# radiocosmology/cora

Hardware: AMD Instinct MI355X
Metric: sky-maps/sec (nside=1024, lmax=2048, 256 freq) (higher is better)
Workload: dtype f64

## Files before the change

### cora_amd/_lib.py

```python
import ctypes
import os
import weakref

import numpy as np

_HERE = os.path.dirname(os.path.abspath(__file__))
LIB_PATH = os.environ.get("CORAHIP_LIB", os.path.join(_HERE, "libcorahip.so"))

c_int, c_double, c_void_p, c_size_t = ctypes.c_int, ctypes.c_double, ctypes.c_void_p, ctypes.c_size_t
c_u64, c_char_p = ctypes.c_uint64, ctypes.c_char_p
PTR = c_void_p

SIGNATURES = {
    "corahip_abi_version": (c_int, []),
    "corahip_abi_minor": (c_int, []),
    "corahip_last_error": (c_char_p, []),
    "corahip_device_count": (c_int, [ctypes.POINTER(c_int)]),
    "corahip_ctx_create": (c_int, [c_int, ctypes.POINTER(c_void_p)]),
    "corahip_ctx_destroy": (c_int, [c_void_p]),
    "corahip_ctx_set_stream": (c_int, [c_void_p, c_void_p]),
    "corahip_ctx_sync": (c_int, [c_void_p]),
    "corahip_timer_begin": (c_int, [c_void_p]),
    "corahip_timer_end": (c_int, [c_void_p, ctypes.POINTER(ctypes.c_float)]),
    "corahip_profile_enable": (c_int, [c_void_p, c_int]),
    "corahip_profile_get": (c_int, [c_void_p, c_char_p, ctypes.POINTER(c_double), ctypes.POINTER(c_int)]),
    "corahip_profile_reset": (c_int, [c_void_p]),
    "corahip_malloc": (c_int, [c_void_p, c_size_t, ctypes.POINTER(c_void_p)]),
    "corahip_free": (c_int, [c_void_p, c_void_p]),
    "corahip_memcpy_h2d": (c_int, [c_void_p, c_void_p, c_void_p, c_size_t]),
    "corahip_memcpy_d2h": (c_int, [c_void_p, c_void_p, c_void_p, c_size_t]),
    "corahip_clarray_table21cm": (c_int, [c_void_p, PTR, PTR, PTR, c_int, c_int, c_double, c_double, c_double,
                                          PTR, PTR, PTR, PTR, c_int, c_int, PTR, PTR, c_int, PTR]),
    "corahip_clarray_table21cm_pairs": (c_int, [c_void_p, PTR, PTR, PTR, c_int, c_int, c_double, c_double, c_double,
                                                PTR, PTR, PTR, PTR, c_int, c_int, PTR, PTR, c_int, c_int, c_int, c_int,
                                                PTR]),
    "corahip_clarray_pairs_finish": (c_int, [c_void_p, PTR, c_int, c_int, c_int, c_int, PTR]),
    "corahip_clarray_tables_pin": (c_int, [c_void_p, PTR, PTR, PTR, c_u64]),
    "corahip_aps_table21cm_points": (c_int, [c_void_p, PTR, PTR, PTR, c_int, c_int, c_double, c_double, c_double,
                                             ctypes.c_long, PTR, PTR, PTR, PTR, PTR, PTR, PTR]),
    "corahip_clarray_separable": (c_int, [c_void_p, PTR, c_int, PTR, c_int, c_int, PTR, PTR]),
    "corahip_romb_reduce": (c_int, [c_void_p, PTR, c_int, c_int, c_int, PTR, PTR]),
    "corahip_factor_batched": (c_int, [c_void_p, PTR, c_int, c_int, c_double, c_double, PTR, PTR]),
    "corahip_normals_philox": (c_int, [c_void_p, c_u64, c_int, c_int, PTR]),
    "corahip_normals_pcg64": (c_int, [c_void_p, ctypes.POINTER(c_u64), ctypes.POINTER(c_u64), ctypes.c_int64, PTR,
                                      ctypes.POINTER(c_u64)]),
    "corahip_normals_mt19937_legacy": (c_int, [c_void_p, c_void_p, ctypes.c_int64, PTR]),
    "corahip_glibc_exp": (c_int, [c_void_p, PTR, ctypes.c_int64, PTR]),
    "corahip_pcg64_advance": (c_int, [ctypes.POINTER(c_u64), ctypes.POINTER(c_u64), c_u64, ctypes.POINTER(c_u64)]),
    "corahip_draw_alm_philox": (c_int, [c_void_p, PTR, PTR, c_u64, c_int, c_int, c_int, c_int, PTR]),
    "corahip_draw_alm_philox_rows": (c_int, [c_void_p, PTR, PTR, c_u64, c_int, c_int, c_int, c_int, PTR]),
    "corahip_draw_alm": (c_int, [c_void_p, PTR, PTR, PTR, c_int, c_int, c_int, c_int, PTR]),
# ... 345 lines not shown

    def to_host(self, t):
        if t.numel() * t.element_size() < self._PINNED_MIN_BYTES:
            return t.cpu().numpy()
        host, done = self.to_host_async(t)
        done.synchronize()
        return host.numpy()

    def pin_tables(self, dd, dv, vv, generation):
        _check(self.lib.corahip_clarray_tables_pin(self.h, self._f64(dd), self._f64(dv), self._f64(vv), c_u64(int(generation))))

    def unpin_tables(self, generation=0):
        if self.h:
            _check(self.lib.corahip_clarray_tables_pin(self.h, None, None, None, c_u64(int(generation))))

    def clarray_table21cm(self, dd, dv, vv, kperpmin, kperpmax, kparmax, chi, pfd, f, b, F, zint, w, log10l):
        nl = log10l.numel()
        out = self.empty((nl, F, F))
        nkperp, nkpar = dd.shape
        _check(self.lib.corahip_clarray_table21cm(
            self.h, self._f64(dd), self._f64(dv), self._f64(vv), nkperp, nkpar, kperpmin, kperpmax, kparmax,
            self._f64(chi), self._f64(pfd), self._f64(f), self._f64(b), F, zint, self._f64(w), self._f64(log10l),
            nl, self._f64(out)))
        return out

    def clarray_table21cm_pairs(self, dd, dv, vv, kperpmin, kperpmax, kparmax, chi, pfd, f, b, F, zint, w, log10l,
                                pair_first, pair_step, l_block, nblocks=None):
        torch = _torch()
        nl = log10l.numel()
        npl = (F * (F + 1) // 2 + pair_step - 1) // pair_step
        nblk = (nl + l_block - 1) // l_block
        if nblocks is not None:
            assert nblocks >= nblk
            nblk = nblocks
        out = torch.zeros((nblk, npl, l_block), dtype=torch.float64, device=self.device)
        nkperp, nkpar = dd.shape
        _check(self.lib.corahip_clarray_table21cm_pairs(
            self.h, self._f64(dd), self._f64(dv), self._f64(vv), nkperp, nkpar, kperpmin, kperpmax, kparmax,
            self._f64(chi), self._f64(pfd), self._f64(f), self._f64(b), F, zint, self._f64(w), self._f64(log10l),
            nl, pair_first, pair_step, l_block, self._f64(out)))
        return out

    def clarray_pairs_finish(self, slabs, F, nl):
        nranks, npl, l_stride = slabs.shape
        assert npl == (F * (F + 1) // 2 + nranks - 1) // nranks and nl <= l_stride
        out = self.empty((nl, F, F))
        _check(self.lib.corahip_clarray_pairs_finish(self.h, self._f64(slabs), F, nranks, l_stride, nl, self._f64(out)))
        return out

    def aps_table21cm_points(self, dd, dv, vv, kperpmin, kperpmax, kparmax, lx, chi1, chi2, cdd, cdv, cvv):
        n = lx.numel()
        out = self.empty((n,))
        nkperp, nkpar = dd.shape
        _check(self.lib.corahip_aps_table21cm_points(
            self.h, self._f64(dd), self._f64(dv), self._f64(vv), nkperp, nkpar, kperpmin, kperpmax, kparmax, n,
            self._f64(lx), self._f64(chi1), self._f64(chi2), self._f64(cdd), self._f64(cdv), self._f64(cvv),
            self._f64(out)))
        return out

    def clarray_separable(self, al, bcov, F, zint, w):
        nl = al.numel()
        out = self.empty((nl, F, F))
# ... 1284 lines not shown
```

### cora_amd/core/maps.py

```python
import numpy as np

from .. import _lib
from ..util import constants
from . import skysim


def _cell_centres(extent, count):
    return (0.5 + np.arange(count)) * (extent / count)


class Map2d(object):

    _geometry_fields = ("x_width", "y_width", "x_num", "y_num", "_nside")

    x_width = y_width = 5.0
    x_num = y_num = 128
    _nside = 128

    @classmethod
    def like_map(cls, mapobj, *args, **kwargs):
        new = cls(*args, **kwargs)
        new._adopt_geometry(mapobj)
        return new

# ... 101 lines not shown
        if self.lmax is None:
            return 3 * self.nside - 1
        return int(self.lmax)

    def _channels(self):
        return np.asarray(self.nu_pixels, dtype=np.float64)

    def getsky(self, rng=None):
        nu = self._channels()
        ctx = _lib.get_context()
        prep = None
        if not isinstance(rng, skysim.DeviceRNG):
            prep = skysim.prepare_numpy_stream(ctx, rng, self._lmax(), len(nu))
        try:
            cl = skysim.clarray_device(self.angular_powerspectrum, self._lmax(), nu,
                                       zromb=self.oversample)
        except BaseException:
            if prep is not None:
                prep.abort()
            raise
        fluct = skysim.mkfullsky_device(cl, self.nside, rng=rng, prepared=prep)
        mean = np.asarray(self.mean_nu(nu), dtype=np.float64) * np.ones(nu.shape)
        if np.any(mean != 0.0):
            fluct += ctx.to_device(mean)[:, None]
        return ctx.to_host(fluct)

    def getpolsky(self, rng=None):
        stokes_i = self.getsky(rng=rng)
        nfreq, npix = stokes_i.shape
        cube = np.zeros((nfreq, 4, npix), dtype=stokes_i.dtype)
        cube[:, 0, :] = stokes_i
        return cube

    def getalms(self, lmax, rng=None):
        cl = skysim.clarray_device(self.angular_powerspectrum, lmax, self._channels())
        return _lib.get_context().to_host(skysim.mkfullsky_device(cl, self.nside, alms=True, rng=rng))
```

### cora_amd/core/skysim.py

```python
import weakref

import numpy as np
import scipy.integrate as si

from .. import _lib
from ..util import nputil
from ..util.nputil import DeviceRNG

_GENERIC_LCHUNK = 8


def romberg_weights(zromb):
    if zromb == 0:
        return np.ones(1)
    zint = 2**zromb + 1
    return si.romb(np.eye(zint), dx=1.0, axis=0) / 2**zromb


def _plan_of(aps):
    obj = getattr(aps, "__self__", None)
    fn = getattr(obj, "_clarray_plan", None)
    return fn(aps) if fn is not None else None


def clarray_device(aps, lmax, zarray, zromb=3, zwidth=None):
    zarray = np.asarray(zarray, dtype=np.float64)
    ctx = _lib.get_context()
    zlen = zarray.size
    if zromb == 0:
        zint = 1
        za = zarray.copy()
    else:
        zsort = np.sort(zarray)
        zhalf = np.abs(zsort[1] - zsort[0]) / 2.0 if zwidth is None else zwidth / 2.0
        zint = 2**zromb + 1
        za = (zarray[:, np.newaxis] + np.linspace(-zhalf, zhalf, zint)[np.newaxis, :]).flatten()
        np.array_split(np.arange(lmax + 1), lmax // 5)
    w = ctx.to_device(romberg_weights(zromb))
    larr = np.arange(lmax + 1, dtype=np.float64)

    plan = _plan_of(aps)
    if plan is not None and plan["kind"] == "table21cm":
        p = plan["prepare"](ctx, za)
        lx = np.log10(np.where(larr == 0.0, 1e-10, larr))
        return ctx.clarray_table21cm(p["dd"], p["dv"], p["vv"], p["kperpmin"], p["kperpmax"], p["kparmax"],
                                     ctx.to_device(p["chi"]), ctx.to_device(p["pfd"]), ctx.to_device(p["f"]),
                                     ctx.to_device(p["b"]), zlen, zint, w, ctx.to_device(lx))
    if plan is not None and plan["kind"] == "separable":
        al, bcov = plan["prepare"](larr.copy(), za)
        return ctx.clarray_separable(ctx.to_device(al), ctx.to_device(bcov), zlen, zint, w)

    import torch

    out = ctx.empty((lmax + 1, zlen, zlen))
    for l0 in range(0, lmax + 1, _GENERIC_LCHUNK):
        lsec = np.arange(l0, min(l0 + _GENERIC_LCHUNK, lmax + 1))
        clt = aps(lsec[:, np.newaxis, np.newaxis].astype(np.float64), za[np.newaxis, :, np.newaxis],
                  za[np.newaxis, np.newaxis, :])
        clt = np.array(np.broadcast_to(clt, (len(lsec), za.size, za.size)), dtype=np.float64, order="C", copy=True)
        out[l0 : l0 + len(lsec)] = ctx.romb_reduce(torch.from_numpy(clt).to(ctx.device), len(lsec), zlen, zint, w)
    return out

# ... 402 lines not shown
```

### cora_amd/csrc/clarray.hip

```cpp
#include "common.h"

#include <cstring>
#include <type_traits>

#define CL_MAXZ 17

#define CL_XS 512
#define CL_LPT 9

__global__ void cl_transpose_kernel(const double *__restrict__ dd, const double *__restrict__ dv,
                                    const double *__restrict__ vv, int nkperp, int nkpar, double *__restrict__ tt) {
    __shared__ double tile[32][33];
    const double *src = blockIdx.z == 0 ? dd : (blockIdx.z == 1 ? dv : vv);
    double *dst = tt + (size_t)blockIdx.z * nkpar * CL_XS;
    const int x0 = blockIdx.y * 32, y0 = blockIdx.x * 32;
    const int tx = threadIdx.x & 31, ty = threadIdx.x >> 5;
    for (int r = ty; r < 32; r += 8) {
        const int x = x0 + r, y = y0 + tx;
        tile[r][tx] = (x < nkperp && y < nkpar) ? src[(size_t)x * nkpar + y] : 0.0;
    }
    __syncthreads();
    for (int r = ty; r < 32; r += 8) {
        const int y = y0 + r, x = x0 + tx;
        if (y < nkpar && x < CL_XS) dst[(size_t)y * CL_XS + x] = (x < nkperp) ? tile[tx][r] : 0.0;
// ... 226 lines not shown
        dd = 4 * xq + (sq & 3);
    } else {
        p -= (long)nfull * CL_BAND;
        int e = n >= CL_BAND ? CL_BAND - 1 : n;
        i = nfull;
        while (p >= e) {
            p -= e;
            e--;
            i++;
        }
        dd = (int)p;
    }
    return make_int2(i, i + CL_BAND * B + dd);
}

__global__ void cl_finish_kernel(const double *__restrict__ scratch, long npairs, int W, long npl, int lstride, int nl,
                                 int F, double *__restrict__ out) {
    __shared__ double tile[32][33];
    const long s0 = (long)blockIdx.x * 32;
    const int l0 = blockIdx.y * 32;
    const int tx = threadIdx.x & 31, ty = threadIdx.x >> 5;
    const long nslot = npl * W;
    for (int r = ty; r < 32; r += 8) {
        const long sl = s0 + r;
        const int l = l0 + tx;
        tile[r][tx] = (sl < nslot && l < nl) ? scratch[(size_t)sl * lstride + l] : 0.0;
    }
    __syncthreads();
    const long sl = s0 + tx;
    const long p = sl < nslot ? (sl % npl) * W + sl / npl : npairs;
    if (p >= npairs) return;
    const int2 ij = pair_of_index(p, F);
    for (int r = ty; r < 32; r += 8) {
        const int l = l0 + r;
        if (l < nl) {
            out[((size_t)l * F + ij.x) * F + ij.y] = tile[tx][r];
        }
    }
}

__global__ void cl_mirror_kernel(double *__restrict__ out, int F) {
    __shared__ double tile[32][33];
    const int nt = (F + 31) / 32;
    int ti = 0, rem = blockIdx.x;
    while (rem >= nt - ti) {
        rem -= nt - ti;
        ti++;
    }
    const int tj = ti + rem;
    double *o = out + (size_t)blockIdx.y * F * F;
    const int tx = threadIdx.x & 31, ty = threadIdx.x >> 5;
    for (int r = ty; r < 32; r += 8) {
        const int i = ti * 32 + r, j = tj * 32 + tx;
        tile[r][tx] = (i < F && j < F) ? o[(size_t)i * F + j] : 0.0;
    }
    __syncthreads();
    for (int r = ty; r < 32; r += 8) {
        const int j = tj * 32 + r, i = ti * 32 + tx;
        if (j < F && i < F && j > i) o[(size_t)j * F + i] = tile[tx][r];
    }
}
static int launch_mirror(corahip_ctx *ctx, double *out, int nl, int F) {
    const int nt = (F + 31) / 32;
    dim3 grid((unsigned)(nt * (nt + 1) / 2), (unsigned)nl);
    cl_mirror_kernel<<<grid, 256, 0, ctx->stream>>>(out, F);
    LAUNCH_CHECK();
    return 0;
}

__global__ void separable_kernel(const double *__restrict__ al, int nl, const double *__restrict__ bcov, int F, int zint,
                                 const double *__restrict__ w, double *__restrict__ out) {
    const long n = (long)nl * F * F;
    const int nz = F * zint;
    for (long q = (long)blockIdx.x * blockDim.x + threadIdx.x; q < n; q += (long)gridDim.x * blockDim.x) {
        const int j = (int)(q % F), i = (int)((q / F) % F);
        const long l = q / ((long)F * F);
        double s = 0.0;
        for (int a = 0; a < zint; a++) {
            double t = 0.0;
            for (int b = 0; b < zint; b++) t += w[b] * bcov[(size_t)(i * zint + a) * nz + j * zint + b];
// ... 97 lines not shown
    ARG_CHECK(ctx != nullptr);
    if (dd == nullptr && generation != 0 && !(ctx->tt_pinned && ctx->tt_pin_gen == generation))
        return 0;
    const bool same = ctx->tt_pinned && dd && ctx->tt_pin[0] == dd && ctx->tt_pin[1] == dv && ctx->tt_pin[2] == vv &&
                      ctx->tt_pin_gen == generation;
    if (same) return 0;
    ctx->tt_pin[0] = dd;
    ctx->tt_pin[1] = dv;
    ctx->tt_pin[2] = vv;
    ctx->tt_pin_gen = generation;
    ctx->tt_pinned = dd != nullptr;
    ctx->tt_valid = false;
    return 0;
}

int corahip_clarray_table21cm(corahip_ctx *ctx, const double *dd, const double *dv, const double *vv, int nkperp,
                              int nkpar, double kperpmin, double kperpmax, double kparmax, const double *chi,
                              const double *pfd, const double *f, const double *b, int F, int zint, const double *w,
                              const double *log10l, int nl, double *out) {
    ARG_CHECK(ctx != nullptr && dd && dv && vv && chi && pfd && f && b && w && log10l && out);
    ARG_CHECK(nkperp >= 2 && nkperp < CL_XS && nkpar >= 2 && F >= 1 && zint >= 1 && zint <= CL_MAXZ && nl >= 1);
    ARG_CHECK(kperpmin > 0 && kperpmax > kperpmin && kparmax > 0);
    StageTimer t(ctx, "clarray");
    const long npairs = (long)F * (F + 1) / 2;
    double *scratch = nullptr;
    int rc;
    if ((rc = corahip_ctx_scratch(ctx, 1, sizeof(double) * (size_t)npairs * nl, (void **)&scratch))) return rc;
    if ((rc = clarray21_pairs(ctx, dd, dv, vv, nkperp, nkpar, kperpmin, kperpmax, kparmax, chi, pfd, f, b, F, zint, w,
                              log10l, nl, 0, 1, npairs, nl, scratch)))
        return rc;
    dim3 grid((unsigned)((npairs + 31) / 32), (nl + 31) / 32);
    cl_finish_kernel<<<grid, 256, 0, ctx->stream>>>(scratch, npairs, 1, npairs, nl, nl, F, out);
    LAUNCH_CHECK();
    return launch_mirror(ctx, out, nl, F);
}

int corahip_clarray_table21cm_pairs(corahip_ctx *ctx, const double *dd, const double *dv, const double *vv, int nkperp,
                                    int nkpar, double kperpmin, double kperpmax, double kparmax, const double *chi,
                                    const double *pfd, const double *f, const double *b, int F, int zint,
                                    const double *w, const double *log10l, int nl, int pair_first, int pair_step,
                                    int l_block, double *out_pairs) {
    ARG_CHECK(ctx != nullptr && dd && dv && vv && chi && pfd && f && b && w && log10l && out_pairs);
    ARG_CHECK(nkperp >= 2 && nkperp < CL_XS && nkpar >= 2 && F >= 1 && zint >= 1 && zint <= CL_MAXZ && nl >= 1);
    ARG_CHECK(kperpmin > 0 && kperpmax > kperpmin && kparmax > 0);
    ARG_CHECK(pair_step >= 1 && pair_first >= 0 && pair_first < pair_step && l_block >= 1);
    StageTimer t(ctx, "clarray");
    const long npairs = (long)F * (F + 1) / 2;
    const long npl = (npairs + pair_step - 1) / pair_step;
    return clarray21_pairs(ctx, dd, dv, vv, nkperp, nkpar, kperpmin, kperpmax, kparmax, chi, pfd, f, b, F, zint, w,
                           log10l, nl, pair_first, pair_step, npl, l_block, out_pairs);
}

int corahip_clarray_pairs_finish(corahip_ctx *ctx, const double *pairs_in, int F, int nranks, int l_stride, int nl,
                                 double *out) {
    ARG_CHECK(ctx != nullptr && pairs_in && out && F >= 1 && nranks >= 1 && nl >= 1 && l_stride >= nl);
    StageTimer t(ctx, "clarray");
    const long npairs = (long)F * (F + 1) / 2;
    const long npl = (npairs + nranks - 1) / nranks;
    dim3 grid((unsigned)((npl * nranks + 31) / 32), (nl + 31) / 32);
    cl_finish_kernel<<<grid, 256, 0, ctx->stream>>>(pairs_in, npairs, nranks, npl, l_stride, nl, F, out);
    LAUNCH_CHECK();
    return launch_mirror(ctx, out, nl, F);
}

int corahip_clarray_separable(corahip_ctx *ctx, const double *al, int nl, const double *bcov, int F, int zint,
                              const double *w, double *out) {
    ARG_CHECK(ctx != nullptr && al && bcov && w && out && nl >= 1 && F >= 1 && zint >= 1);
    StageTimer t(ctx, "clarray");
    const long n = (long)nl * F * F;
    separable_kernel<<<(int)std::min<long>((n + 255) / 256, 4096), 256, 0, ctx->stream>>>(al, nl, bcov, F, zint, w, out);
    LAUNCH_CHECK();
    return 0;
}

int corahip_romb_reduce(corahip_ctx *ctx, const double *clt, int nl, int F, int zint, const double *w, double *out) {
    ARG_CHECK(ctx != nullptr && clt && w && out && nl >= 1 && F >= 1 && zint >= 1);
    StageTimer t(ctx, "clarray");
// ... 23 lines not shown
```

### cora_amd/csrc/common.h

```cpp
#pragma once
#include <hip/hip_runtime.h>

#include <cstdarg>
#include <cstdint>
#include <cstdio>
#include <map>
#include <string>
#include <type_traits>
#include <vector>

#include "../../include/corahip.h"

void corahip_set_error(const char *fmt, ...);

struct corahip_prof_entry {
    double total_ms = 0.0;
    int launches = 0;
};

struct corahip_pending_event {
    std::string name;
    hipEvent_t e0, e1;
};

struct corahip_linefft_plan {
    int n = 0, P = 0, logP = 0, blu = 0;
    int Pct = 0;
    double2 *filt_ct = nullptr;
    double2 *tw = nullptr;
    double2 *chirp = nullptr;
    double2 *filt = nullptr;
    double2 *rtw = nullptr;
};

#define CORAHIP_NSCRATCH 12
struct corahip_ctx {
    int device = 0;
    hipStream_t stream = nullptr;
    hipStream_t stream2 = nullptr;
    hipEvent_t ev_fork = nullptr, ev_join = nullptr;
    int *k5_tickets = nullptr;
    unsigned *draw_slot_tab = nullptr;
    int draw_slot_lmax = -1;
    bool mt_plist_ready = false;
    hipStream_t gen_stream = nullptr;
    hipEvent_t ev_ring[8] = {};
    const void *draw_pending = nullptr;
    hipEvent_t t0 = nullptr, t1 = nullptr;
    bool profile = false;
    std::map<std::string, corahip_prof_entry> prof;
// ... 123 lines not shown
```

### cora_amd/csrc/factor.hip

```cpp
#include "common.h"
#include "jacobi_sweep.h"

#include <algorithm>
#include <vector>

#define CH_NB 32

__global__ void __launch_bounds__(256)
chol_kernel(const double *__restrict__ C, int F, double jitter_rel, double *__restrict__ T,
            int32_t *__restrict__ info) {
    extern __shared__ __attribute__((aligned(16))) double lds[];
    double *D = lds;
    double *PA = lds + CH_NB * (CH_NB + 1);
    double *PB = PA + 64 * (CH_NB + 1);
    double *red = PB + 64 * (CH_NB + 1);
    int *flag = reinterpret_cast<int *>(red + 256);

    const int tid = threadIdx.x;
    const size_t off = (size_t)blockIdx.x * F * F;
    const double *A = C + off;
    double *Tl = T + off;

    double dmax = -INFINITY;
    for (int i = tid; i < F; i += 256) dmax = fmax(dmax, A[(size_t)i * F + i]);
// ... 123 lines not shown
    }
    if (tid == 0) info[blockIdx.x] = *flag;
}

#define CHM_S 34
#ifndef CHM_STAMPS
#define CHM_STAMPS 0
#endif
#if CHM_STAMPS
__device__ unsigned long long g_chm_stamps[8];
#define CSTAMP(k) { unsigned long long _t; asm volatile("s_memtime %0\n\ts_waitcnt lgkmcnt(0)" : "=s"(_t)::"memory"); c_acc[k] += _t - c_last; c_last = _t; }
#else
#define CSTAMP(k)
#endif

template <bool TALL>
__global__ void __launch_bounds__(256)
chol_ll_kernel(const double *__restrict__ C, int F, double jitter_rel, double *__restrict__ T,
               int32_t *__restrict__ info) {
    extern __shared__ __attribute__((aligned(16))) double lds[];
    double *D = lds;
    double *red = lds + CH_NB * (CH_NB + 1);
    int *flag = reinterpret_cast<int *>(red + 256);
    double *rdiag = red + 256 + 2;
    double *stage = rdiag + CH_NB;

    const int tid = threadIdx.x, lane = tid & 63, wave = tid >> 6;
    const int ri = lane & 15, kq = lane >> 4;
    const size_t off = (size_t)blockIdx.x * F * F;
    const double *A = C + off;
    double *Tl = T + off;
    double *PA = stage + (size_t)wave * (TALL ? 1 : 2) * 32 * CHM_S, *PB = PA + 32 * CHM_S;
    double *PBS = stage + 4 * 32 * CHM_S;

// ... 508 lines not shown
                        if (p < jj) s[p & 3] = fma(-x[p], D[jj * (CH_NB + 1) + p], s[p & 3]);
                    x[jj] = ((s[0] + s[1]) + (s[2] + s[3])) * rdiag[jj];
                }
            }
#pragma unroll
            for (int jj = 0; jj < CH_NB; jj += 2) *reinterpret_cast<double2 *>(row + jj) = make_double2(x[jj], x[jj + 1]);
        }
        group_sync();
    }
    if (wgl == 0 && tid == 0) {
        info[mat0 + mi] = failed;
        xcc_max[mi] = same_xcc ? 0x100 : 0x200;
    }
}

__global__ void __launch_bounds__(JAC_NT)
jacobi_root_kernel(const double *__restrict__ C, const int32_t *__restrict__ list, int F, double jitter_rel,
                   double eig_thresh, double *__restrict__ Wall, double *__restrict__ Vall,
                   double *__restrict__ T) {
    extern __shared__ __attribute__((aligned(16))) double lds[];
    double *cs = lds;
    double *red = lds + 2 * (F / 2 + 1);
    double *ev = red + JAC_NT;
    int *order = reinterpret_cast<int *>(ev + F);
    const int tid = threadIdx.x;
    const int l = list[blockIdx.x];
    const double *A = C + (size_t)l * F * F;
    double *W = Wall + (size_t)blockIdx.x * F * F;
    double *V = Vall + (size_t)blockIdx.x * F * F;
    double *Tl = T + (size_t)l * F * F;

    double dmax = -INFINITY;
    for (int i = tid; i < F; i += JAC_NT) dmax = fmax(dmax, A[(size_t)i * F + i]);
    red[tid] = dmax;
    __syncthreads();
    for (int s = JAC_NT / 2; s > 0; s >>= 1) {
        if (tid < s) red[tid] = fmax(red[tid], red[tid + s]);
        __syncthreads();
    }
    const double jit = red[0] * jitter_rel;
    __syncthreads();
    for (long q = tid; q < (long)F * F; q += JAC_NT) {
        const int i = (int)(q / F), j = (int)(q % F);
        const double v = (j <= i) ? A[(size_t)i * F + j] : A[(size_t)j * F + i];
        W[q] = v + (i == j ? jit : 0.0);
        V[q] = (i == j) ? 1.0 : 0.0;
    }
    jacobi_sweeps(W, V, F, cs, red);
    for (int i = tid; i < F; i += JAC_NT) ev[i] = W[(size_t)i * F + i];
    __syncthreads();
    double emax = -INFINITY;
    for (int i = tid; i < F; i += JAC_NT) emax = fmax(emax, ev[i]);
    red[tid] = emax;
    __syncthreads();
    for (int s = JAC_NT / 2; s > 0; s >>= 1) {
        if (tid < s) red[tid] = fmax(red[tid], red[tid + s]);
        __syncthreads();
    }
    emax = red[0];
    __syncthreads();
    jacobi_rank(ev, order, F);
    __syncthreads();
    for (long q = tid; q < (long)F * F; q += JAC_NT) {
        const int i = (int)(q / F), j = (int)(q % F);
        double e = ev[j];
        if (e < emax * eig_thresh) e = 0.0;
        Tl[(size_t)i * F + order[j]] = V[q] * sqrt(e);
    }
}

extern "C" int corahip_factor_batched(corahip_ctx *ctx, const double *C, int nl, int F, double jitter_rel,
                                      double eig_thresh, double *T, int32_t *info) {
    ARG_CHECK(ctx != nullptr && C != nullptr && T != nullptr && info != nullptr);
    ARG_CHECK(nl >= 1 && F >= 1);
    StageTimer t(ctx, "factor");
    if (F >= 64 && (F % 2) == 0) {
        const bool tall = F >= 384;
        const size_t shm = sizeof(double) * (CH_NB * (CH_NB + 1) + 256 + 2 + CH_NB + (tall ? 6 : 8) * 32 * CHM_S) + 16;
        const char *coop_env = getenv("CORAHIP_K2_COOP");
        const int nblk = (F + 31) / 32;
        const int G = (nblk + 3) / 4;
        int nrem = 0;
        if (tall && (F % 32) == 0 && !(coop_env && atoi(coop_env) == 0) && !CHM_STAMPS) {
            const int slots = 2 * ctx->num_cu;
            const int r = nl % slots;
            if (nl > slots && r > 0 && ((r + 7) / 8) * 8 * G <= ctx->num_cu && r <= 16) nrem = r;
            if (coop_env && atoi(coop_env) == 2 && ((nl + 7) / 8) * 8 * G <= ctx->num_cu) nrem = nl;
        }
        const size_t shm2 = sizeof(double) * (CH_NB * (CH_NB + 1) + 256 + 2 + CH_NB + 8 * 32 * CHM_S) + 16;
        if (nrem > 0) {
            HIP_TRY(hipFuncSetAttribute((const void *)chol_coop_kernel, hipFuncAttributeMaxDynamicSharedMemorySize, (int)shm2));
            int per_cu = 0;
            HIP_TRY(hipOccupancyMaxActiveBlocksPerMultiprocessor(&per_cu, (const void *)chol_coop_kernel, 256, shm2));
            if ((long)per_cu * ctx->num_cu < (long)((nrem + 7) / 8) * 8 * G) nrem = 0;
        }
        const int nmain = nl - nrem;
        if (tall) {
// ... 22 lines not shown
        {
            unsigned long long hs[8], z[8] = {0};
            HIP_TRY(hipStreamSynchronize(ctx->stream));
            HIP_TRY(hipMemcpyFromSymbol(hs, HIP_SYMBOL(g_chm_stamps), sizeof(hs)));
            const double per = 1.0 / (double)std::max<unsigned long long>(hs[7], 1);
            fprintf(stderr, "K2 F=%d nl=%d tall=%d: cycles/wave  A %.0f  bar %.0f  B %.0f  bar %.0f  C %.0f  bar %.0f\n", F, nl, (int)tall,
                    hs[0] * per, hs[1] * per, hs[2] * per, hs[3] * per, hs[4] * per, hs[5] * per);
            HIP_TRY(hipMemcpyToSymbol(HIP_SYMBOL(g_chm_stamps), z, sizeof(z)));
        }
#endif
    } else {
        const size_t shm = sizeof(double) * (CH_NB * (CH_NB + 1) + 2 * 64 * (CH_NB + 1) + 256) + 16;
        chol_kernel<<<nl, 256, shm, ctx->stream>>>(C, F, jitter_rel, T, info);
        LAUNCH_CHECK();
    }
    std::vector<int32_t> hinfo(nl);
    HIP_TRY(hipMemcpyAsync(hinfo.data(), info, sizeof(int32_t) * nl, hipMemcpyDeviceToHost, ctx->stream));
    HIP_TRY(hipStreamSynchronize(ctx->stream));
    {
        bool redo = false;
        for (int l = 0; l < nl; l++)
            if (hinfo[l] == 3) {
                const size_t shm = sizeof(double) * (CH_NB * (CH_NB + 1) + 256 + 2 + CH_NB + 6 * 32 * CHM_S) + 16;
                chol_ll_kernel<true><<<1, 256, shm, ctx->stream>>>(C + (size_t)l * F * F, F, jitter_rel, T + (size_t)l * F * F, info + l);
                LAUNCH_CHECK();
                redo = true;
            }
        if (redo) {
            HIP_TRY(hipMemcpyAsync(hinfo.data(), info, sizeof(int32_t) * nl, hipMemcpyDeviceToHost, ctx->stream));
            HIP_TRY(hipStreamSynchronize(ctx->stream));
        }
    }
    std::vector<int32_t> list;
    for (int l = 0; l < nl; l++)
        if (hinfo[l] != 0) list.push_back(l);
    if (list.empty()) return 0;
    const size_t per = (size_t)2 * F * F * sizeof(double);
    const size_t batch = std::max<size_t>(1, std::min<size_t>(list.size(), ((size_t)1 << 31) / per));
    int32_t *dlist = nullptr;
    double *scratch = nullptr;
    HIP_TRY(hipMalloc((void **)&dlist, sizeof(int32_t) * list.size()));
    HIP_TRY(hipMalloc((void **)&scratch, per * batch));
    HIP_TRY(hipMemcpyAsync(dlist, list.data(), sizeof(int32_t) * list.size(), hipMemcpyHostToDevice, ctx->stream));
    const size_t shm = sizeof(double) * (2 * (F / 2 + 1) + JAC_NT + F) + sizeof(int) * (F + 4) + 16;
    for (size_t b0 = 0; b0 < list.size(); b0 += batch) {
        const int nb = (int)std::min(batch, list.size() - b0);
        jacobi_root_kernel<<<nb, JAC_NT, shm, ctx->stream>>>(C, dlist + b0, F, jitter_rel, eig_thresh, scratch,
                                                         scratch + (size_t)nb * F * F, T);
        LAUNCH_CHECK();
    }
    HIP_TRY(hipStreamSynchronize(ctx->stream));
    (void)hipFree(dlist);
    (void)hipFree(scratch);
    return 0;
}
```

### cora_amd/parallel.py

```python
from dataclasses import dataclass


@dataclass
class ShardPlan:
    rank: int
    world: int
    l_lo: int
    l_hi: int
    l_shard: int
    l_pad: int
    nu0: int
    nnu: int
    L: int = 0
    chunks: tuple = ()


def fold_chunks(F, rank, world):
    if F % (2 * world) or (F // (2 * world)) % 4:
        raise ValueError("fold=True needs F divisible by 8 * world (F = %d, world = %d)" % (F, world))
    c = F // (2 * world)
    return ((rank * c, c), ((2 * world - 1 - rank) * c, c))


def fold_permutation(F, world):
# ... 324 lines not shown
            self._emulated = (Tf, inf, rows)
            nl0 = sp.l_hi - sp.l_lo
            self._emu_C = ctx.empty((nl0, F, F))
            for l0 in range(0, nl0, lc):
                Cc = ctx.empty((min(lc, nl0 - l0), F, F)).normal_()
                self._emu_C[l0:l0 + Cc.shape[0]].copy_(Cc @ Cc.transpose(1, 2) + eye)
                del Cc

    def _chan_index(self):
        import torch

        if getattr(self, "_chan_idx", None) is None:
            self._chan_idx = torch.as_tensor(self.channels, device=self.ctx.device)
        return self._chan_idx

    def _clarray_local(self):
        ctx = self.ctx
        if self._sep is not None:
            return ctx.clarray_separable(self._sep[0], self._sep[1], self.F, self.zint, self.w)
        return ctx.clarray_table21cm(*self._tabs, *self._k1, self.F, self.zint, self.w, self._lx)

    def _separable_factors(self):
        import torch

        ctx = self.ctx
        one = torch.ones((1,), dtype=torch.float64, device=ctx.device)
        bbar = ctx.clarray_separable(one, self._sep[1], self.F, self.zint, self.w)
        tb, ib = ctx.factor_batched(bbar)
        rows = tb[0].index_select(0, self._chan_index())
        T = torch.sqrt(self._sep[2])[:, None, None] * rows[None, :, :]
        info = ib.expand(self.L).contiguous()
        return T.contiguous(), info, True

    def _clarray_pairs(self, first, step):
        return self.ctx.clarray_table21cm_pairs(*self._tabs, *self._k1, self.F, self.zint, self.w, self._lx, first, step,
# ... 23 lines not shown
            return Tr, ia, True
        Ta, ia = allgather_factors(T, info, sp)
        return Ta, ia, False

    def factors(self):
        ctx, sp = self.ctx, self.plan
        if self._sep is not None:
            return self._separable_factors()
        if self.emulate_world > 1:
            N = self.emulate_world
            if self.pair_sharded:
                slab = self._clarray_pairs(N - 1, N)
                C = ctx.clarray_pairs_finish(slab.new_zeros((N,) + tuple(slab.shape[1:])), self.F, sp.l_hi - sp.l_lo)
                del C
            else:
                self._clarray_local()
            ctx.factor_batched(self._emu_C)
            return self._emulated
        if not self.distributed:
            T, info = ctx.factor_batched(self._clarray_local())
            return T, info, False
        if self.pair_sharded:
            mine = exchange_pair_slabs(self._clarray_pairs(self.rank, self.world), sp)
            T, info = ctx.factor_batched(ctx.clarray_pairs_finish(mine, self.F, sp.l_hi - sp.l_lo))
            Tr, ia = exchange_factor_rows(T, info, sp)
            return Tr, ia, True
        T, info = ctx.factor_batched(self._clarray_local())
        Ta, ia = allgather_factors(T, info, sp)
        return Ta, ia, False

    def draw(self, seed, factors=None, out=None):
        ctx = self.ctx
        out = self.alm_buf if out is None else out
        T, info, rows = factors if factors is not None else self.factors()
        if rows and self.folded:
# ... 203 lines not shown
```

### include/corahip.h

```cpp
#ifndef CORAHIP_H
#define CORAHIP_H

#include <stddef.h>
#include <stdint.h>

#ifdef __cplusplus
extern "C" {
#endif

#define CORAHIP_ABI_VERSION 1
#define CORAHIP_ABI_MINOR 12

#define CORAHIP_EINVAL (-1)
#define CORAHIP_ENOMEM (-2)
#define CORAHIP_ESTATE (-3)

typedef struct corahip_ctx corahip_ctx;
typedef struct corahip_sht_plan corahip_sht_plan;

int corahip_abi_version(void);
int corahip_abi_minor(void);
const char *corahip_last_error(void);
int corahip_device_count(int *count);
int corahip_ctx_create(int device_id, corahip_ctx **ctx);
// ... 13 lines not shown


int corahip_clarray_table21cm(corahip_ctx *ctx, const double *dd, const double *dv, const double *vv,
                              int nkperp, int nkpar, double kperpmin, double kperpmax, double kparmax,
                              const double *chi, const double *pfd, const double *f, const double *b,
                              int F, int zint, const double *w, const double *log10l, int nl,
                              double *out);

int corahip_clarray_table21cm_pairs(corahip_ctx *ctx, const double *dd, const double *dv, const double *vv,
                                    int nkperp, int nkpar, double kperpmin, double kperpmax, double kparmax,
                                    const double *chi, const double *pfd, const double *f, const double *b,
                                    int F, int zint, const double *w, const double *log10l, int nl,
                                    int pair_first, int pair_step, int l_block, double *out_pairs);
int corahip_clarray_pairs_finish(corahip_ctx *ctx, const double *pairs_in, int F, int nranks, int l_stride,
                                 int nl, double *out);

int corahip_clarray_tables_pin(corahip_ctx *ctx, const double *dd, const double *dv, const double *vv,
                               uint64_t generation);

int corahip_aps_table21cm_points(corahip_ctx *ctx, const double *dd, const double *dv, const double *vv,
                                 int nkperp, int nkpar, double kperpmin, double kperpmax, double kparmax,
                                 long n, const double *lx, const double *chi1, const double *chi2,
                                 const double *cdd, const double *cdv, const double *cvv, double *out);

int corahip_clarray_separable(corahip_ctx *ctx, const double *al, int nl, const double *bcov, int F,
                              int zint, const double *w, double *out);

int corahip_romb_reduce(corahip_ctx *ctx, const double *clt, int nl, int F, int zint, const double *w,
                        double *out);

// ... 219 lines not shown
```

Before: 3203.

## Fuse clarray finish and mirror, add lower-only output, move factor fallbacks on-device

Replaces the separate finish-scatter and mirror kernels with one tiled kernel that gathers pair slots straight into (l,F,F) blocks through swizzled LDS, optionally writing only the lower triangle that the Cholesky factorization reads. The factor path drops its host round-trip on the info array: the tall-Cholesky redo becomes a device-side guarded launch, and the Jacobi fallback becomes a persistent work-stealing kernel that scans info on the GPU and uses cached context scratch instead of hipMalloc/hipFree. The aim is to remove a full extra pass over the C array, cut global-memory traffic, and eliminate host syncs and allocations per call. In exchange, the fallback kernel always launches and scans info, and callers that asked for lower=True get an upper triangle that is left unwritten.

```diff
diff --git a/cora_amd/_lib.py b/cora_amd/_lib.py
--- a/cora_amd/_lib.py
+++ b/cora_amd/_lib.py
@@ -35,6 +35,9 @@
                                                 PTR, PTR, PTR, PTR, c_int, c_int, PTR, PTR, c_int, c_int, c_int, c_int,
                                                 PTR]),
     "corahip_clarray_pairs_finish": (c_int, [c_void_p, PTR, c_int, c_int, c_int, c_int, PTR]),
+    "corahip_clarray_table21cm_lower": (c_int, [c_void_p, PTR, PTR, PTR, c_int, c_int, c_double, c_double, c_double,
+                                                PTR, PTR, PTR, PTR, c_int, c_int, PTR, PTR, c_int, PTR]),
+    "corahip_clarray_pairs_finish_lower": (c_int, [c_void_p, PTR, c_int, c_int, c_int, c_int, PTR]),
     "corahip_clarray_tables_pin": (c_int, [c_void_p, PTR, PTR, PTR, c_u64]),
     "corahip_aps_table21cm_points": (c_int, [c_void_p, PTR, PTR, PTR, c_int, c_int, c_double, c_double, c_double,
                                              ctypes.c_long, PTR, PTR, PTR, PTR, PTR, PTR, PTR]),
@@ -410,11 +413,12 @@
         if self.h:
             _check(self.lib.corahip_clarray_tables_pin(self.h, None, None, None, c_u64(int(generation))))
 
-    def clarray_table21cm(self, dd, dv, vv, kperpmin, kperpmax, kparmax, chi, pfd, f, b, F, zint, w, log10l):
+    def clarray_table21cm(self, dd, dv, vv, kperpmin, kperpmax, kparmax, chi, pfd, f, b, F, zint, w, log10l,
+                          lower=False, out=None):
         nl = log10l.numel()
-        out = self.empty((nl, F, F))
+        out = self._clarray_out(out, nl, F)
         nkperp, nkpar = dd.shape
-        _check(self.lib.corahip_clarray_table21cm(
+        _check((self.lib.corahip_clarray_table21cm_lower if lower else self.lib.corahip_clarray_table21cm)(
             self.h, self._f64(dd), self._f64(dv), self._f64(vv), nkperp, nkpar, kperpmin, kperpmax, kparmax,
             self._f64(chi), self._f64(pfd), self._f64(f), self._f64(b), F, zint, self._f64(w), self._f64(log10l),
             nl, self._f64(out)))
@@ -437,11 +441,18 @@
             nl, pair_first, pair_step, l_block, self._f64(out)))
         return out
 
-    def clarray_pairs_finish(self, slabs, F, nl):
+    def clarray_pairs_finish(self, slabs, F, nl, lower=False, out=None):
         nranks, npl, l_stride = slabs.shape
         assert npl == (F * (F + 1) // 2 + nranks - 1) // nranks and nl <= l_stride
-        out = self.empty((nl, F, F))
-        _check(self.lib.corahip_clarray_pairs_finish(self.h, self._f64(slabs), F, nranks, l_stride, nl, self._f64(out)))
+        out = self._clarray_out(out, nl, F)
+        fn = self.lib.corahip_clarray_pairs_finish_lower if lower else self.lib.corahip_clarray_pairs_finish
+        _check(fn(self.h, self._f64(slabs), F, nranks, l_stride, nl, self._f64(out)))
+        return out
+
+    def _clarray_out(self, out, nl, F):
+        if out is None:
+            return self.empty((nl, F, F))
+        assert tuple(out.shape) == (nl, F, F) and out.is_contiguous()
         return out
 
     def aps_table21cm_points(self, dd, dv, vv, kperpmin, kperpmax, kparmax, lx, chi1, chi2, cdd, cdv, cvv):
diff --git a/cora_amd/core/maps.py b/cora_amd/core/maps.py
--- a/cora_amd/core/maps.py
+++ b/cora_amd/core/maps.py
@@ -139,7 +139,7 @@
             prep = skysim.prepare_numpy_stream(ctx, rng, self._lmax(), len(nu))
         try:
             cl = skysim.clarray_device(self.angular_powerspectrum, self._lmax(), nu,
-                                       zromb=self.oversample)
+                                       zromb=self.oversample, lower=True)
         except BaseException:
             if prep is not None:
                 prep.abort()
@@ -158,5 +158,5 @@
         return cube
 
     def getalms(self, lmax, rng=None):
-        cl = skysim.clarray_device(self.angular_powerspectrum, lmax, self._channels())
+        cl = skysim.clarray_device(self.angular_powerspectrum, lmax, self._channels(), lower=True)
         return _lib.get_context().to_host(skysim.mkfullsky_device(cl, self.nside, alms=True, rng=rng))
diff --git a/cora_amd/core/skysim.py b/cora_amd/core/skysim.py
--- a/cora_amd/core/skysim.py
+++ b/cora_amd/core/skysim.py
@@ -23,7 +23,7 @@
     return fn(aps) if fn is not None else None
 
 
-def clarray_device(aps, lmax, zarray, zromb=3, zwidth=None):
+def clarray_device(aps, lmax, zarray, zromb=3, zwidth=None, lower=False):
     zarray = np.asarray(zarray, dtype=np.float64)
     ctx = _lib.get_context()
     zlen = zarray.size
@@ -45,7 +45,7 @@
         lx = np.log10(np.where(larr == 0.0, 1e-10, larr))
         return ctx.clarray_table21cm(p["dd"], p["dv"], p["vv"], p["kperpmin"], p["kperpmax"], p["kparmax"],
                                      ctx.to_device(p["chi"]), ctx.to_device(p["pfd"]), ctx.to_device(p["f"]),
-                                     ctx.to_device(p["b"]), zlen, zint, w, ctx.to_device(lx))
+                                     ctx.to_device(p["b"]), zlen, zint, w, ctx.to_device(lx), lower=lower)
     if plan is not None and plan["kind"] == "separable":
         al, bcov = plan["prepare"](larr.copy(), za)
         return ctx.clarray_separable(ctx.to_device(al), ctx.to_device(bcov), zlen, zint, w)
diff --git a/cora_amd/csrc/clarray.hip b/cora_amd/csrc/clarray.hip
--- a/cora_amd/csrc/clarray.hip
+++ b/cora_amd/csrc/clarray.hip
@@ -264,56 +264,90 @@
     return make_int2(i, i + CL_BAND * B + dd);
 }
 
-__global__ void cl_finish_kernel(const double *__restrict__ scratch, long npairs, int W, long npl, int lstride, int nl,
-                                 int F, double *__restrict__ out) {
-    __shared__ double tile[32][33];
-    const long s0 = (long)blockIdx.x * 32;
-    const int l0 = blockIdx.y * 32;
-    const int tx = threadIdx.x & 31, ty = threadIdx.x >> 5;
-    const long nslot = npl * W;
-    for (int r = ty; r < 32; r += 8) {
-        const long sl = s0 + r;
-        const int l = l0 + tx;
-        tile[r][tx] = (sl < nslot && l < nl) ? scratch[(size_t)sl * lstride + l] : 0.0;
-    }
-    __syncthreads();
-    const long sl = s0 + tx;
-    const long p = sl < nslot ? (sl % npl) * W + sl / npl : npairs;
-    if (p >= npairs) return;
-    const int2 ij = pair_of_index(p, F);
-    for (int r = ty; r < 32; r += 8) {
-        const int l = l0 + r;
-        if (l < nl) {
-            out[((size_t)l * F + ij.x) * F + ij.y] = tile[tx][r];
-        }
-    }
-}
-
-__global__ void cl_mirror_kernel(double *__restrict__ out, int F) {
-    __shared__ double tile[32][33];
+__host__ __device__ static inline long index_of_pair(int i, int j, int F, int B, long boff) {
+    const int n = F - CL_BAND * B, dd = j - i - CL_BAND * B;
+    const int nfull = n >= CL_BAND ? n - (CL_BAND - 1) : 0;
+    if (i < nfull) return boff + 8L * (4 * i + (dd & 3)) + (dd >> 2);
+    const int e0 = n >= CL_BAND ? CL_BAND - 1 : n, k = i - nfull;
+    return boff + (long)nfull * CL_BAND + (long)k * e0 - (long)k * (k - 1) / 2 + dd;
+}
+
+#define CLF_L 8
+#define CLF_NCH 4
+#define CLF_RP (8 / CLF_L)
+#define CLF_NK (32 / CLF_RP)
+__device__ __forceinline__ int clf_idx(int lc, int ii, int jj) { return lc * 1024 + ii * 32 + (jj ^ ii ^ ((lc & 3) << 3)); }
+template <bool LOWER>
+__global__ void __launch_bounds__(256)
+cl_finish_kernel(const double *__restrict__ scratch, long npairs, int W, long npl, int lstride, int nl, int F,
+                 double *__restrict__ out) {
+    __shared__ double tile[CLF_L * 1024];
     const int nt = (F + 31) / 32;
     int ti = 0, rem = blockIdx.x;
     while (rem >= nt - ti) {
         rem -= nt - ti;
         ti++;
     }
-    const int tj = ti + rem;
-    double *o = out + (size_t)blockIdx.y * F * F;
-    const int tx = threadIdx.x & 31, ty = threadIdx.x >> 5;
-    for (int r = ty; r < 32; r += 8) {
-        const int i = ti * 32 + r, j = tj * 32 + tx;
-        tile[r][tx] = (i < F && j < F) ? o[(size_t)i * F + j] : 0.0;
-    }
-    __syncthreads();
-    for (int r = ty; r < 32; r += 8) {
-        const int j = tj * 32 + r, i = ti * 32 + tx;
-        if (j < F && i < F && j > i) o[(size_t)j * F + i] = tile[tx][r];
-    }
-}
-static int launch_mirror(corahip_ctx *ctx, double *out, int nl, int F) {
+    const int tj = ti + rem, D = tj - ti;
+    long boff = 0;
+    for (int B = 0; B < D; B++) boff += cl_band_count(F - CL_BAND * B);
+    const long boff1 = D > 0 ? cl_band_count(F - CL_BAND * (D - 1)) : 0;
+    const int tid = threadIdx.x;
+    const int lc = tid % CLF_L, jj = (tid / CLF_L) & 31, ksub = tid / (CLF_L * 32), j = tj * 32 + jj;
+    int slot[CLF_NK];
+#pragma unroll
+    for (int k = 0; k < CLF_NK; k++) {
+        const int ii = k * CLF_RP + ksub, i = ti * 32 + ii;
+        slot[k] = -1;
+        if (i < F && j < F && j >= i) {
+            const bool own = jj >= ii;
+            const long p = index_of_pair(i, j, F, own ? D : D - 1, own ? boff : boff - boff1);
+            if (p < npairs) slot[k] = (int)((p % W) * npl + p / W);
+        }
+    }
+    const int tx = tid & 31, ty = tid >> 5;
+    const int lbase = blockIdx.y * (CLF_L * CLF_NCH);
+    double v[CLF_NK];
+    auto request = [&](int l0) {
+        if (l0 + lc < nl) {
+#pragma unroll
+            for (int k = 0; k < CLF_NK; k++)
+                if (slot[k] >= 0) v[k] = scratch[(size_t)slot[k] * lstride + l0 + lc];
+        }
+    };
+    request(lbase);
+    for (int c = 0; c < CLF_NCH; c++) {
+        const int l0 = lbase + c * CLF_L;
+        if (l0 >= nl) break;
+        if (l0 + lc < nl) {
+#pragma unroll
+            for (int k = 0; k < CLF_NK; k++)
+                if (slot[k] >= 0) tile[clf_idx(lc, k * CLF_RP + ksub, jj)] = v[k];
+        }
+        __syncthreads();
+        if (c + 1 < CLF_NCH) request(l0 + CLF_L);
+        for (int q = 0; q < CLF_L && l0 + q < nl; q++) {
+            double *o = out + (size_t)(l0 + q) * F * F;
+#pragma unroll
+            for (int r = ty; r < 32; r += 8) {
+                if (!LOWER) {
+                    const int i = ti * 32 + r, jw = tj * 32 + tx;
+                    if (i < F && jw < F && jw >= i) o[(size_t)i * F + jw] = tile[clf_idx(q, r, tx)];
+                }
+                const int jr = tj * 32 + r, i = ti * 32 + tx;
+                if (jr < F && i < F && (LOWER ? jr >= i : jr > i)) o[(size_t)jr * F + i] = tile[clf_idx(q, tx, r)];
+            }
+        }
+        __syncthreads();
+    }
+}
+static int launch_finish(corahip_ctx *ctx, const double *scratch, long npairs, int W, long npl, int lstride, int nl, int F,
+                         bool lower, double *out) {
+    ARG_CHECK(npl * W < ((long)1 << 31));
     const int nt = (F + 31) / 32;
-    dim3 grid((unsigned)(nt * (nt + 1) / 2), (unsigned)nl);
-    cl_mirror_kernel<<<grid, 256, 0, ctx->stream>>>(out, F);
+    dim3 grid((unsigned)(nt * (nt + 1) / 2), (unsigned)((nl + CLF_L * CLF_NCH - 1) / (CLF_L * CLF_NCH)));
+    if (lower) cl_finish_kernel<true><<<grid, 256, 0, ctx->stream>>>(scratch, npairs, W, npl, lstride, nl, F, out);
+    else cl_finish_kernel<false><<<grid, 256, 0, ctx->stream>>>(scratch, npairs, W, npl, lstride, nl, F, out);
     LAUNCH_CHECK();
     return 0;
 }
@@ -441,10 +475,10 @@
     return 0;
 }
 
-int corahip_clarray_table21cm(corahip_ctx *ctx, const double *dd, const double *dv, const double *vv, int nkperp,
-                              int nkpar, double kperpmin, double kperpmax, double kparmax, const double *chi,
-                              const double *pfd, const double *f, const double *b, int F, int zint, const double *w,
-                              const double *log10l, int nl, double *out) {
+static int clarray21_full(corahip_ctx *ctx, const double *dd, const double *dv, const double *vv, int nkperp,
+                          int nkpar, double kperpmin, double kperpmax, double kparmax, const double *chi,
+                          const double *pfd, const double *f, const double *b, int F, int zint, const double *w,
+                          const double *log10l, int nl, bool lower, double *out) {
     ARG_CHECK(ctx != nullptr && dd && dv && vv && chi && pfd && f && b && w && log10l && out);
     ARG_CHECK(nkperp >= 2 && nkperp < CL_XS && nkpar >= 2 && F >= 1 && zint >= 1 && zint <= CL_MAXZ && nl >= 1);
     ARG_CHECK(kperpmin > 0 && kperpmax > kperpmin && kparmax > 0);
@@ -456,10 +490,23 @@
     if ((rc = clarray21_pairs(ctx, dd, dv, vv, nkperp, nkpar, kperpmin, kperpmax, kparmax, chi, pfd, f, b, F, zint, w,
                               log10l, nl, 0, 1, npairs, nl, scratch)))
         return rc;
-    dim3 grid((unsigned)((npairs + 31) / 32), (nl + 31) / 32);
-    cl_finish_kernel<<<grid, 256, 0, ctx->stream>>>(scratch, npairs, 1, npairs, nl, nl, F, out);
-    LAUNCH_CHECK();
-    return launch_mirror(ctx, out, nl, F);
+    return launch_finish(ctx, scratch, npairs, 1, npairs, nl, nl, F, lower, out);
+}
+
+int corahip_clarray_table21cm(corahip_ctx *ctx, const double *dd, const double *dv, const double *vv, int nkperp,
+                              int nkpar, double kperpmin, double kperpmax, double kparmax, const double *chi,
+                              const double *pfd, const double *f, const double *b, int F, int zint, const double *w,
+                              const double *log10l, int nl, double *out) {
+    return clarray21_full(ctx, dd, dv, vv, nkperp, nkpar, kperpmin, kperpmax, kparmax, chi, pfd, f, b, F, zint, w, log10l, nl,
+                          false, out);
+}
+
+int corahip_clarray_table21cm_lower(corahip_ctx *ctx, const double *dd, const double *dv, const double *vv, int nkperp,
+                                    int nkpar, double kperpmin, double kperpmax, double kparmax, const double *chi,
+                                    const double *pfd, const double *f, const double *b, int F, int zint, const double *w,
+                                    const double *log10l, int nl, double *out) {
+    return clarray21_full(ctx, dd, dv, vv, nkperp, nkpar, kperpmin, kperpmax, kparmax, chi, pfd, f, b, F, zint, w, log10l, nl,
+                          true, out);
 }
 
 int corahip_clarray_table21cm_pairs(corahip_ctx *ctx, const double *dd, const double *dv, const double *vv, int nkperp,
@@ -478,16 +525,23 @@
                            log10l, nl, pair_first, pair_step, npl, l_block, out_pairs);
 }
 
-int corahip_clarray_pairs_finish(corahip_ctx *ctx, const double *pairs_in, int F, int nranks, int l_stride, int nl,
-                                 double *out) {
+static int pairs_finish(corahip_ctx *ctx, const double *pairs_in, int F, int nranks, int l_stride, int nl, bool lower,
+                        double *out) {
     ARG_CHECK(ctx != nullptr && pairs_in && out && F >= 1 && nranks >= 1 && nl >= 1 && l_stride >= nl);
     StageTimer t(ctx, "clarray");
     const long npairs = (long)F * (F + 1) / 2;
     const long npl = (npairs + nranks - 1) / nranks;
-    dim3 grid((unsigned)((npl * nranks + 31) / 32), (nl + 31) / 32);
-    cl_finish_kernel<<<grid, 256, 0, ctx->stream>>>(pairs_in, npairs, nranks, npl, l_stride, nl, F, out);
-    LAUNCH_CHECK();
-    return launch_mirror(ctx, out, nl, F);
+    return launch_finish(ctx, pairs_in, npairs, nranks, npl, l_stride, nl, F, lower, out);
+}
+
+int corahip_clarray_pairs_finish(corahip_ctx *ctx, const double *pairs_in, int F, int nranks, int l_stride, int nl,
+                                 double *out) {
+    return pairs_finish(ctx, pairs_in, F, nranks, l_stride, nl, false, out);
+}
+
+int corahip_clarray_pairs_finish_lower(corahip_ctx *ctx, const double *pairs_in, int F, int nranks, int l_stride, int nl,
+                                       double *out) {
+    return pairs_finish(ctx, pairs_in, F, nranks, l_stride, nl, true, out);
 }
 
 int corahip_clarray_separable(corahip_ctx *ctx, const double *al, int nl, const double *bcov, int F, int zint,
diff --git a/cora_amd/csrc/common.h b/cora_amd/csrc/common.h
--- a/cora_amd/csrc/common.h
+++ b/cora_amd/csrc/common.h
@@ -33,7 +33,7 @@
     double2 *rtw = nullptr;
 };
 
-#define CORAHIP_NSCRATCH 12
+#define CORAHIP_NSCRATCH 13
 struct corahip_ctx {
     int device = 0;
     hipStream_t stream = nullptr;
diff --git a/cora_amd/csrc/factor.hip b/cora_amd/csrc/factor.hip
--- a/cora_amd/csrc/factor.hip
+++ b/cora_amd/csrc/factor.hip
@@ -161,10 +161,13 @@
 #define CSTAMP(k)
 #endif
 
-template <bool TALL>
+template <bool TALL, bool REDO = false>
 __global__ void __launch_bounds__(256)
 chol_ll_kernel(const double *__restrict__ C, int F, double jitter_rel, double *__restrict__ T,
                int32_t *__restrict__ info) {
+    if constexpr (REDO) {
+        if (info[blockIdx.x] != 3) return;
+    }
     extern __shared__ __attribute__((aligned(16))) double lds[];
     double *D = lds;
     double *red = lds + CH_NB * (CH_NB + 1);
@@ -703,58 +706,92 @@
     }
 }
 
+__device__ static void jacobi_root_one(const double *__restrict__ A, double *__restrict__ Tl, double *__restrict__ W,
+                                       double *__restrict__ V, int F, double jitter_rel, double eig_thresh, double *cs,
+                                       double *red, double *ev, int *order) {
+    const int tid = threadIdx.x;
+    double dmax = -INFINITY;
+    for (int i = tid; i < F; i += JAC_NT) dmax = fmax(dmax, A[(size_t)i * F + i]);
+    red[tid] = dmax;
+    __syncthreads();
+    for (int s = JAC_NT / 2; s > 0; s >>= 1) {
+        if (tid < s) red[tid] = fmax(red[tid], red[tid + s]);
+        __syncthreads();
+    }
+    const double jit = red[0] * jitter_rel;
+    __syncthreads();
+    for (long q = tid; q < (long)F * F; q += JAC_NT) {
+        const int i = (int)(q / F), j = (int)(q % F);
+        const double v = (j <= i) ? A[(size_t)i * F + j] : A[(size_t)j * F + i];
+        W[q] = v + (i == j ? jit : 0.0);
+        V[q] = (i == j) ? 1.0 : 0.0;
+    }
+    jacobi_sweeps(W, V, F, cs, red);
+    for (int i = tid; i < F; i += JAC_NT) ev[i] = W[(size_t)i * F + i];
+    __syncthreads();
+    double emax = -INFINITY;
+    for (int i = tid; i < F; i += JAC_NT) emax = fmax(emax, ev[i]);
+    red[tid] = emax;
+    __syncthreads();
+    for (int s = JAC_NT / 2; s > 0; s >>= 1) {
+        if (tid < s) red[tid] = fmax(red[tid], red[tid + s]);
+        __syncthreads();
+    }
+    emax = red[0];
+    __syncthreads();
+    jacobi_rank(ev, order, F);
+    __syncthreads();
+    for (long q = tid; q < (long)F * F; q += JAC_NT) {
+        const int i = (int)(q / F), j = (int)(q % F);
+        double e = ev[j];
+        if (e < emax * eig_thresh) e = 0.0;
+        Tl[(size_t)i * F + order[j]] = V[q] * sqrt(e);
+    }
+}
+
 __global__ void __launch_bounds__(JAC_NT)
-jacobi_root_kernel(const double *__restrict__ C, const int32_t *__restrict__ list, int F, double jitter_rel,
-                   double eig_thresh, double *__restrict__ Wall, double *__restrict__ Vall,
-                   double *__restrict__ T) {
+jacobi_root_kernel(const double *__restrict__ C, const int32_t *__restrict__ info, int *__restrict__ cursor, int nl, int F,
+                   double jitter_rel, double eig_thresh, double *__restrict__ slots, double *__restrict__ T) {
     extern __shared__ __attribute__((aligned(16))) double lds[];
     double *cs = lds;
     double *red = lds + 2 * (F / 2 + 1);
     double *ev = red + JAC_NT;
     int *order = reinterpret_cast<int *>(ev + F);
+    int *cnt = order + F;
+    int *pick = cnt + JAC_NT;
     const int tid = threadIdx.x;
-    const int l = list[blockIdx.x];
-    const double *A = C + (size_t)l * F * F;
-    double *W = Wall + (size_t)blockIdx.x * F * F;
-    double *V = Vall + (size_t)blockIdx.x * F * F;
-    double *Tl = T + (size_t)l * F * F;
-
-    double dmax = -INFINITY;
-    for (int i = tid; i < F; i += JAC_NT) dmax = fmax(dmax, A[(size_t)i * F + i]);
-    red[tid] = dmax;
-    __syncthreads();
-    for (int s = JAC_NT / 2; s > 0; s >>= 1) {
-        if (tid < s) red[tid] = fmax(red[tid], red[tid + s]);
-        __syncthreads();
-    }
-    const double jit = red[0] * jitter_rel;
-    __syncthreads();
-    for (long q = tid; q < (long)F * F; q += JAC_NT) {
-        const int i = (int)(q / F), j = (int)(q % F);
-        const double v = (j <= i) ? A[(size_t)i * F + j] : A[(size_t)j * F + i];
-        W[q] = v + (i == j ? jit : 0.0);
-        V[q] = (i == j) ? 1.0 : 0.0;
-    }
-    jacobi_sweeps(W, V, F, cs, red);
-    for (int i = tid; i < F; i += JAC_NT) ev[i] = W[(size_t)i * F + i];
-    __syncthreads();
-    double emax = -INFINITY;
-    for (int i = tid; i < F; i += JAC_NT) emax = fmax(emax, ev[i]);
-    red[tid] = emax;
-    __syncthreads();
-    for (int s = JAC_NT / 2; s > 0; s >>= 1) {
-        if (tid < s) red[tid] = fmax(red[tid], red[tid + s]);
-        __syncthreads();
-    }
-    emax = red[0];
-    __syncthreads();
-    jacobi_rank(ev, order, F);
-    __syncthreads();
-    for (long q = tid; q < (long)F * F; q += JAC_NT) {
-        const int i = (int)(q / F), j = (int)(q % F);
-        double e = ev[j];
-        if (e < emax * eig_thresh) e = 0.0;
-        Tl[(size_t)i * F + order[j]] = V[q] * sqrt(e);
+    double *W = slots + (size_t)blockIdx.x * 2 * F * F;
+    double *V = W + (size_t)F * F;
+
+    const int seg = (nl + JAC_NT - 1) / JAC_NT;
+    const int seg0 = min(tid * seg, nl), seg1 = min(seg0 + seg, nl);
+    int mine = 0;
+    for (int l = seg0; l < seg1; l++) mine += info[l] != 0;
+    cnt[tid] = mine;
+    __syncthreads();
+    for (int o = 1; o < JAC_NT; o <<= 1) {
+        const int v = tid >= o ? cnt[tid - o] : 0;
+        __syncthreads();
+        cnt[tid] += v;
+        __syncthreads();
+    }
+    const int nfail = cnt[JAC_NT - 1], before = cnt[tid] - mine;
+    if (nfail == 0) return;
+
+    for (;;) {
+        __syncthreads();
+        if (tid == 0) pick[1] = atomicAdd(cursor, 1);
+        __syncthreads();
+        const int ticket = pick[1];
+        if (ticket >= nfail) return;
+        if (ticket >= before && ticket < before + mine) {
+            int seen = before;
+            for (int l = seg0; l < seg1; l++)
+                if (info[l] != 0 && seen++ == ticket) pick[0] = l;
+        }
+        __syncthreads();
+        const int l = pick[0];
+        jacobi_root_one(C + (size_t)l * F * F, T + (size_t)l * F * F, W, V, F, jitter_rel, eig_thresh, cs, red, ev, order);
     }
 }
 
@@ -763,13 +800,13 @@
     ARG_CHECK(ctx != nullptr && C != nullptr && T != nullptr && info != nullptr);
     ARG_CHECK(nl >= 1 && F >= 1);
     StageTimer t(ctx, "factor");
+    int nrem = 0;
     if (F >= 64 && (F % 2) == 0) {
         const bool tall = F >= 384;
         const size_t shm = sizeof(double) * (CH_NB * (CH_NB + 1) + 256 + 2 + CH_NB + (tall ? 6 : 8) * 32 * CHM_S) + 16;
         const char *coop_env = getenv("CORAHIP_K2_COOP");
         const int nblk = (F + 31) / 32;
         const int G = (nblk + 3) / 4;
-        int nrem = 0;
         if (tall && (F % 32) == 0 && !(coop_env && atoi(coop_env) == 0) && !CHM_STAMPS) {
             const int slots = 2 * ctx->num_cu;
             const int r = nl % slots;
@@ -822,43 +859,22 @@
         chol_kernel<<<nl, 256, shm, ctx->stream>>>(C, F, jitter_rel, T, info);
         LAUNCH_CHECK();
     }
-    std::vector<int32_t> hinfo(nl);
-    HIP_TRY(hipMemcpyAsync(hinfo.data(), info, sizeof(int32_t) * nl, hipMemcpyDeviceToHost, ctx->stream));
-    HIP_TRY(hipStreamSynchronize(ctx->stream));
-    {
-        bool redo = false;
-        for (int l = 0; l < nl; l++)
-            if (hinfo[l] == 3) {
-                const size_t shm = sizeof(double) * (CH_NB * (CH_NB + 1) + 256 + 2 + CH_NB + 6 * 32 * CHM_S) + 16;
-                chol_ll_kernel<true><<<1, 256, shm, ctx->stream>>>(C + (size_t)l * F * F, F, jitter_rel, T + (size_t)l * F * F, info + l);
-                LAUNCH_CHECK();
-                redo = true;
-            }
-        if (redo) {
-            HIP_TRY(hipMemcpyAsync(hinfo.data(), info, sizeof(int32_t) * nl, hipMemcpyDeviceToHost, ctx->stream));
-            HIP_TRY(hipStreamSynchronize(ctx->stream));
-        }
-    }
-    std::vector<int32_t> list;
-    for (int l = 0; l < nl; l++)
-        if (hinfo[l] != 0) list.push_back(l);
-    if (list.empty()) return 0;
+    if (nrem > 0) {
+        const size_t shm = sizeof(double) * (CH_NB * (CH_NB + 1) + 256 + 2 + CH_NB + 6 * 32 * CHM_S) + 16;
+        const size_t off = (size_t)(nl - nrem) * F * F;
+        HIP_TRY(hipFuncSetAttribute((const void *)chol_ll_kernel<true, true>, hipFuncAttributeMaxDynamicSharedMemorySize, (int)shm));
+        chol_ll_kernel<true, true><<<nrem, 256, shm, ctx->stream>>>(C + off, F, jitter_rel, T + off, info + (nl - nrem));
+        LAUNCH_CHECK();
+    }
     const size_t per = (size_t)2 * F * F * sizeof(double);
-    const size_t batch = std::max<size_t>(1, std::min<size_t>(list.size(), ((size_t)1 << 31) / per));
-    int32_t *dlist = nullptr;
-    double *scratch = nullptr;
-    HIP_TRY(hipMalloc((void **)&dlist, sizeof(int32_t) * list.size()));
-    HIP_TRY(hipMalloc((void **)&scratch, per * batch));
-    HIP_TRY(hipMemcpyAsync(dlist, list.data(), sizeof(int32_t) * list.size(), hipMemcpyHostToDevice, ctx->stream));
-    const size_t shm = sizeof(double) * (2 * (F / 2 + 1) + JAC_NT + F) + sizeof(int) * (F + 4) + 16;
-    for (size_t b0 = 0; b0 < list.size(); b0 += batch) {
-        const int nb = (int)std::min(batch, list.size() - b0);
-        jacobi_root_kernel<<<nb, JAC_NT, shm, ctx->stream>>>(C, dlist + b0, F, jitter_rel, eig_thresh, scratch,
-                                                         scratch + (size_t)nb * F * F, T);
-        LAUNCH_CHECK();
-    }
-    HIP_TRY(hipStreamSynchronize(ctx->stream));
-    (void)hipFree(dlist);
-    (void)hipFree(scratch);
+    const int G = (int)std::max<size_t>(1, std::min<size_t>(std::min(nl, ctx->num_cu), ((size_t)1 << 31) / per));
+    char *ws = nullptr;
+    int rc = corahip_ctx_scratch(ctx, 12, 256 + per * G, (void **)&ws);
+    if (rc) return rc;
+    HIP_TRY(hipMemsetAsync(ws, 0, sizeof(int), ctx->stream));
+    const size_t shm = sizeof(double) * (2 * (F / 2 + 1) + JAC_NT + F) + sizeof(int) * (F + JAC_NT + 4) + 16;
+    jacobi_root_kernel<<<G, JAC_NT, shm, ctx->stream>>>(C, info, reinterpret_cast<int *>(ws), nl, F, jitter_rel, eig_thresh,
+                                                       reinterpret_cast<double *>(ws + 256), T);
+    LAUNCH_CHECK();
     return 0;
 }
diff --git a/cora_amd/parallel.py b/cora_amd/parallel.py
--- a/cora_amd/parallel.py
+++ b/cora_amd/parallel.py
@@ -362,11 +362,11 @@
             self._chan_idx = torch.as_tensor(self.channels, device=self.ctx.device)
         return self._chan_idx
 
-    def _clarray_local(self):
+    def _clarray_local(self, lower=False):
         ctx = self.ctx
         if self._sep is not None:
             return ctx.clarray_separable(self._sep[0], self._sep[1], self.F, self.zint, self.w)
-        return ctx.clarray_table21cm(*self._tabs, *self._k1, self.F, self.zint, self.w, self._lx)
+        return ctx.clarray_table21cm(*self._tabs, *self._k1, self.F, self.zint, self.w, self._lx, lower=lower)
 
     def _separable_factors(self):
         import torch
@@ -420,11 +420,11 @@
                 C = ctx.clarray_pairs_finish(slab.new_zeros((N,) + tuple(slab.shape[1:])), self.F, sp.l_hi - sp.l_lo)
                 del C
             else:
-                self._clarray_local()
+                self._clarray_local(lower=True)
             ctx.factor_batched(self._emu_C)
             return self._emulated
         if not self.distributed:
-            T, info = ctx.factor_batched(self._clarray_local())
+            T, info = ctx.factor_batched(self._clarray_local(lower=True))
             return T, info, False
         if self.pair_sharded:
             mine = exchange_pair_slabs(self._clarray_pairs(self.rank, self.world), sp)
diff --git a/include/corahip.h b/include/corahip.h
--- a/include/corahip.h
+++ b/include/corahip.h
@@ -51,6 +51,14 @@
                                     int pair_first, int pair_step, int l_block, double *out_pairs);
 int corahip_clarray_pairs_finish(corahip_ctx *ctx, const double *pairs_in, int F, int nranks, int l_stride,
                                  int nl, double *out);
+
+int corahip_clarray_table21cm_lower(corahip_ctx *ctx, const double *dd, const double *dv, const double *vv,
+                                    int nkperp, int nkpar, double kperpmin, double kperpmax, double kparmax,
+                                    const double *chi, const double *pfd, const double *f, const double *b,
+                                    int F, int zint, const double *w, const double *log10l, int nl,
+                                    double *out);
+int corahip_clarray_pairs_finish_lower(corahip_ctx *ctx, const double *pairs_in, int F, int nranks, int l_stride,
+                                       int nl, double *out);
 
 int corahip_clarray_tables_pin(corahip_ctx *ctx, const double *dd, const double *dv, const double *vv,
                                uint64_t generation);
```

After: 3220, median of 6. No clear change (+0.5%).
